# WinnerBy/PreGANPlus

Hardware: AMD Instinct MI355X
Metric: host-windows/sec (detect+diagnose+generate) (higher is better)
Workload: dtype fp32; 1 GPU; C2: PreGAN+ batched inference, 50 hosts x W=3 x 3 resources, 65536 windows per GPU, fp32; windows_per_gpu=65536, parallelism=dp1 (independent windows)

## Files before the change

### preganplus_amd/csrc/pgp_capi.hip

```cpp
#include <hip/hip_runtime.h>

#include <string>

#include "../../include/preganplus.h"
#include "pgp_device.hpp"
#include "pgp_pack.hpp"
#include "pgp_repack.hpp"
#include "pgp_train.hpp"
#include "pgp_tune.hpp"
#include "pgp_tunef.hpp"
#include "pgp_tunedp.hpp"

#include <vector>

using namespace pgp;

struct pgp_model {
  int H = 0, K = 0;
  bool fpe = false;
  bool loaded = false;
  float* d_frags = nullptr;
  float* d_decb = nullptr;
  float* d_encb = nullptr;
  bool enc_split = true;
  bool dec_split = true;
  float* d_ganb = nullptr;
  bool gan_split = true;
  float* d_tab = nullptr;
  float* d_gtab = nullptr;
  float* d_gat = nullptr;
  double* d_pscr = nullptr;
  int cap = 0;
  float* d_agg = nullptr;
  float* d_lat = nullptr;
  float* d_emb = nullptr;
};

namespace {
thread_local std::string g_err;
int fail(int code, const std::string& msg) {
  g_err = msg;
  return code;
}
#define HIPCHK(x)                                                                                  \
  do {                                                                                             \
    hipError_t e_ = (x);                                                                           \
    if (e_ != hipSuccess) return fail(PGP_ERR_HIP, std::string(#x) + ": " + hipGetErrorString(e_)); \
// ... 147 lines not shown
  if (batch < 0) return fail(PGP_ERR_ARG, "negative batch");
  if (stage < -1 || stage > 3) return fail(PGP_ERR_ARG, "bad stage");
  if (batch == 0) return PGP_OK;
  const bool all = stage == -1;
  if (((all || stage == 0) && !windows) ||
      ((all || stage == 2) && (!logits || !protos || !cls || !any_anom)) ||
      ((all || stage == 3) && (!sched || !probs || !keep_orig || !final_target || !gen_target)))
    return fail(PGP_ERR_ARG, "NULL input/output pointer");
  if (batch > m->cap) {
    const int rc = reserve(m, batch);
    if (rc) return rc;
  }
  FwdArgs a{};
  a.B = batch;
  a.H = m->H;
  a.K = m->K;
  a.windows = windows;
  a.sched = sched;
  a.agg = m->d_agg;
  a.lat = m->d_lat;
  a.emb = m->d_emb;
  a.frags = m->d_frags;
  a.decb = m->dec_split ? m->d_decb : nullptr;
  a.encb = m->enc_split ? m->d_encb : nullptr;
  a.ganb = m->gan_split ? m->d_ganb : nullptr;
  a.tab = m->d_tab;
  a.gtab = m->d_gtab;
  a.gat = m->d_gat;
  a.logits = logits;
  a.protos = protos;
  a.cls = cls;
  a.any_anom = any_anom;
  a.probs = probs;
  a.keep = keep_orig;
  a.final_t = final_target;
  a.gen_t = gen_target;
  a.latent = latent;
  hipStream_t st = reinterpret_cast<hipStream_t>(stream);
  if (all || stage == 0) HIPCHK(launch_gat(a, st));
  if (all || stage == 1) HIPCHK(launch_encoder(a, st));
  if (all || stage == 2) HIPCHK(launch_decoder(a, st));
  if (all || stage == 3) HIPCHK(launch_gan(a, st));
  return PGP_OK;
}

int pgp_forward(pgp_model* m, int batch, const float* windows, const float* sched, float* logits, float* protos,
                int* cls, int* any_anom, float* probs, int* keep_orig, int* final_target, int* gen_target,
                float* latent, void* stream) {
  return pgp_forward_stage(m, -1, batch, windows, sched, logits, protos, cls, any_anom, probs, keep_orig,
                           final_target, gen_target, latent, stream);
}

int pgp_forward_fpe_stage(pgp_model* m, int stage, int batch, const float* windows, const float* h0,
                          const float* sched, float* scores, float* protos, int* cls, int* any_anom, float* probs,
                          int* keep_orig, int* final_target, int* gen_target, void* stream) {
  if (!m) return fail(PGP_ERR_ARG, "NULL model");
  if (!m->loaded) return fail(PGP_ERR_STATE, "weights not loaded");
  if (!m->fpe) return fail(PGP_ERR_STATE, "not an FPE model: use pgp_forward");
  if (batch < 0) return fail(PGP_ERR_ARG, "negative batch");
  if (stage < -1 || stage > 1) return fail(PGP_ERR_ARG, "bad stage");
  if (batch == 0) return PGP_OK;
  const bool all = stage == -1;
  if (((all || stage == 0) && (!windows || !h0 || !scores || !protos || !cls || !any_anom)) ||
// ... 48 lines not shown
  HIPCHK(launch_decide(batch, n_hosts, keep_orig, final_target, cur_host, moves, hosts_from,
                       reinterpret_cast<hipStream_t>(stream)));
  return PGP_OK;
}

int pgp_embedding(int n_hosts, int batch, const float* logits, const float* protos, float* emb, void* stream) {
  if (n_hosts < 1 || batch < 0) return fail(PGP_ERR_ARG, "bad embedding arguments");
  if (batch == 0) return PGP_OK;
  if (!logits || !protos || !emb) return fail(PGP_ERR_ARG, "NULL input/output pointer");
  HIPCHK(launch_embed((long)batch * n_hosts, logits, protos, emb, reinterpret_cast<hipStream_t>(stream)));
  return PGP_OK;
}

int pgp_decoder_split(pgp_model* m, int on) {
  if (!m) return fail(PGP_ERR_ARG, "NULL model");
  if (m->fpe || decoder_split_floats(m->H) == 0)
    return on ? fail(PGP_ERR_UNSUPPORTED, "split-bf16 decoder not compiled for this model / host count") : PGP_OK;
  m->dec_split = on != 0;
  return PGP_OK;
}

int pgp_encoder_split(pgp_model* m, int on) {
  if (!m) return fail(PGP_ERR_ARG, "NULL model");
  if (m->fpe || encoder_split_floats(m->H) == 0)
    return on ? fail(PGP_ERR_UNSUPPORTED, "split-bf16 encoder not compiled for this model / host count") : PGP_OK;
  m->enc_split = on != 0;
  return PGP_OK;
}

int pgp_gan_split(pgp_model* m, int on) {
  if (!m) return fail(PGP_ERR_ARG, "NULL model");
  if (gan_split_floats(m->H) == 0)
    return on ? fail(PGP_ERR_UNSUPPORTED, "split-bf16 GAN kernel not compiled for this host count") : PGP_OK;
  m->gan_split = on != 0;
  return PGP_OK;
}

int pgp_schedule_onehot(int n_hosts, int batch, const unsigned char* idx, float* sched, void* stream) {
  if (n_hosts < 1 || n_hosts > 255 || batch < 0) return fail(PGP_ERR_ARG, "bad schedule_onehot arguments");
  if (batch == 0) return PGP_OK;
  if (!idx || !sched) return fail(PGP_ERR_ARG, "NULL input/output pointer");
  HIPCHK(launch_onehot(n_hosts, (long)batch * n_hosts, idx, sched, reinterpret_cast<hipStream_t>(stream)));
  return PGP_OK;
}

namespace {
bool master_offsets(int H, long* tr, long* gen, long* disc, long* all) {
  switch (H) {
#define CASE(h)                     \
// ... 415 lines not shown
```

### preganplus_amd/csrc/pgp_device.hpp

```cpp
#pragma once
#include <hip/hip_runtime.h>

#include <atomic>
#include <string>

#include "pgp_layout.hpp"

namespace pgp {

typedef float f32x4 __attribute__((ext_vector_type(4)));
typedef float f32x2 __attribute__((ext_vector_type(2)));

constexpr int kMaxProtos = 64;

inline int device_cus() {
  static std::atomic<int> cached[64];
  int dev = 0;
  if (hipGetDevice(&dev) != hipSuccess || dev < 0 || dev >= 64) return 256;
  int n = cached[dev].load(std::memory_order_relaxed);
  if (n == 0) {
    if (hipDeviceGetAttribute(&n, hipDeviceAttributeMultiprocessorCount, dev) != hipSuccess || n <= 0) n = 256;
    cached[dev].store(n, std::memory_order_relaxed);
  }
  return n;
// ... 29 lines not shown
  const float* windows;
  const float* h0;
  const float* tab;
  float* scores;
  float* protos;
  int* cls;
  int* any_anom;
  float* emb;
};
hipError_t launch_fpe(int H, const FpeArgs& a, hipStream_t st);
int fpe_param_count(int H);
hipError_t launch_fpe_step(int n_hosts, const float* win, const float* h0, const int* y, const int* cls,
                           const float* P, float* G, int K, double* state, double update_min, double decay,
                           double* loss, hipStream_t st);
hipError_t launch_fpe_forward_many(int n_hosts, int n, const float* wins, const float* h0s, const float* P,
                                   double* probs, double* protos, hipStream_t st);

hipError_t launch_decide(int B, int C, const int* keep, const int* target, const int* cur, int* moves,
                         int* hosts_from, hipStream_t st);
hipError_t launch_embed(long n, const float* logits, const float* protos, float* emb, hipStream_t st);
hipError_t launch_onehot(int H, long rows, const unsigned char* idx, float* sched, hipStream_t st);

hipError_t launch_gat(const FwdArgs& a, hipStream_t st);
hipError_t launch_encoder(const FwdArgs& a, hipStream_t st);
hipError_t launch_decoder(const FwdArgs& a, hipStream_t st);
long decoder_split_floats(int H);
hipError_t launch_decoder_split(int H, const float* frags, float* decb, hipStream_t st);
long encoder_split_floats(int H);
hipError_t launch_encoder_split(int H, const float* frags, float* encb, hipStream_t st);
hipError_t launch_gan(const FwdArgs& a, hipStream_t st);
long gan_split_floats(int H);
hipError_t launch_gan_split_derive(int H, const float* frags, float* planes, hipStream_t st);
hipError_t launch_gan_split(const FwdArgs& a, hipStream_t st);

struct AdamArgs;
struct AdamFuse;
long gan_workspace_floats(int H, int B);
int gan_plan_slices(int H, int B);
hipError_t launch_adamw(const AdamArgs& a, hipStream_t st);
bool gan1_supported(int H);
hipError_t launch_gan1_forward(int H, const float* emb, const float* sched, const float* Pg, const float* Pd,
                               float* row, float* ns, float* probs, hipStream_t st);
hipError_t launch_gan1_step(int H, const float* target, float* Pg, float* Pd, float* Gg, float* Gd, float* row,
                            const AdamArgs& ad, const AdamArgs& ag, float* probs_gen, float* probs_after,
                            hipStream_t st);

hipError_t launch_gan_fwd(int H, int B, const float* emb, const float* sched, const float* Pg, const float* Pd,
// ... 135 lines not shown
```

### preganplus_amd/csrc/pgp_encoder.hip

```cpp
#include "pgp_device.hpp"

namespace pgp {
namespace {

constexpr int kEncWaves = 4;
constexpr int kEnc16Waves = 4, kEnc16EU = 2;
template <int H>
constexpr bool tail_res() { return Geo<H>::TAIL; }
constexpr int kEncTailWaves = 8;
template <int H>
constexpr int enc_waves() { return H <= 16 ? kEnc16Waves : tail_res<H>() ? kEncTailWaves : kEncWaves; }
template <int H>
constexpr int NW_STAGE() { return enc_waves<H>(); }

#ifndef PGP_ENC_PIPE
#define PGP_ENC_PIPE 1
#endif
constexpr bool kEncPipe = PGP_ENC_PIPE != 0;
#ifndef PGP_ENC_PIPE_F32
#define PGP_ENC_PIPE_F32 0
#endif
constexpr bool kEncPipeF32 = PGP_ENC_PIPE_F32 != 0;

template <int H>
struct EncS {
  using G = Geo<H>;
  static constexpr int NBD = cdiv(G::KQ_D, 2);
  static constexpr int NBF = G::KQ_F / 2;
  static constexpr int F1S = G::MT_F * NBD * 3;
  static constexpr int F2S = G::MT_X * NBF * 3;
  static constexpr int FFN = F1S + F2S;
  static constexpr int L0F = 0;
  static constexpr int L1A = FFN;
  static constexpr int L1F = L1A + G::P_F1;
  static constexpr int GROUPS = L1F + FFN;
  static constexpr int STREAM = GROUPS * G::FQ;
  static constexpr long SIZE = STREAM;
};

template <int H, bool SPLIT = false>
struct EncLds {
  static constexpr bool TRES = tail_res<H>();
  static constexpr int RES0 = TRES ? Geo<H>::st_begin(Geo<H>::NST - 1) : 0;
  static constexpr int STREAM = SPLIT ? EncS<H>::STREAM : (kLayers * Geo<H>::LAYER_G - RES0) * Geo<H>::FQ;
  static constexpr bool RESIDENT = TRES || STREAM * 4 <= 32 * 1024;
// ... 112 lines not shown
        a = ld4(A + (m * KQ + q4) * 256 + lane * 4);
      }
      f32x4 rw[NR];
      if (m == 0) {
#pragma unroll
        for (int n = 0; n < NR; ++n) rw[n] = ld4(RW + ((n * KQ + q4) * 4 + g) * 4);
      }
#pragma unroll
      for (int e = 0; e < 4; ++e)
        if (4 * q4 + e < KS) {
#pragma unroll
          for (int w = 0; w < 3; ++w) {
            acc[m][w] = mfma(a[e], Bx[q4][w][e], acc[m][w]);
            if (m == 0) {
#pragma unroll
              for (int n = 0; n < NR; ++n) racc[n][w] = fmaf(rw[n][e], Bx[q4][w][e], racc[n][w]);
            }
          }
        }
    }
  prio_valu();
}

template <int NR>
PGP_DEV void rows_finish(float (&r)[NR][3]) {
  float* f = &r[0][0];
#pragma unroll
  for (int i = 0; i + 1 < 3 * NR; i += 2) xsum2(f[i], f[i + 1]);
  if constexpr ((3 * NR) % 2) f[3 * NR - 1] = xsum(f[3 * NR - 1], true);
}

template <int NR>
PGP_DEV float rows_pick(const float (&r)[NR][3], int w) {
  float v[NR];
#pragma unroll
  for (int n = 0; n < NR; ++n) v[n] = r[n][w];
  return xsum_rows<NR>(v);
}

template <int NR>
PGP_DEV void zero_rows(float (&r)[NR][3]) {
#pragma unroll
  for (int n = 0; n < NR; ++n)
#pragma unroll
    for (int w = 0; w < 3; ++w) r[n][w] = 0.f;
}
// ... 135 lines not shown
PGP_DEV void qkv_fold(f32x4 (&acc)[NM][3], int T0, int n, const float* tab, const float (&ba)[3], int lane, int g) {
  using G = Geo<H>;
#pragma unroll
  for (int m = 0; m < NM; ++m)
    if (m < n) {
      const float a = tab[G::T_F0 + (T0 + m) * 64 + lane];
#pragma unroll
      for (int w = 0; w < 3; ++w)
        acc[m][w] = mfma(a, ba[w], ld4(tab + G::T_F0B + (w * 3 * G::NQT + T0 + m) * 16 + 4 * g));
    }
}
template <int H>
PGP_DEV float row_fold_part(int m, int n, int w, const float* tab, const float (&ba)[3], int g) {
  using G = Geo<H>;
  const float t = tab[G::T_F0R + (m * G::SR + n) * 4 + g];
  return (g < 3 ? t : 0.f) * ba[w];
}
template <int H>
PGP_DEV float row_fold_bias(int m, int n, int w, const float* tab) {
  using G = Geo<H>;
  return tab[G::T_F0RB + w * 3 * G::SR + m * G::SR + n];
}

template <int H, bool F0, bool SPLIT>
PGP_DEV void encoder_layer_tail(f32x4 (&X)[Geo<H>::MT_D][3], Ring<H, SPLIT>& ring, const float* TL, int lane,
                                const float* tab, const float (&ba)[3], const float (&xv)[3][3]) {
  using G = Geo<H>;
  constexpr int TQ = G::TQ, SR = G::SR, HF = G::HF;
  const int g = lane >> 4;
  constexpr bool BIL = F0;
  f32x4 QK[BIL ? 1 : 2 * TQ][3];
  float qr[SR][3], kr[SR][3];
  if constexpr (BIL) {
  } else {
#pragma unroll
    for (int m = 0; m < 2 * TQ; ++m) {
      const f32x4 bias = ld4(TL + G::TL_QKV + m * 16 + 4 * g);
#pragma unroll
      for (int w = 0; w < 3; ++w) QK[m][w] = bias;
    }
    float qkr[2 * SR][3];
    zero_rows(qkr);
    gemm3_rows<2 * TQ, G::KQ_D, G::KS_D, G::MT_D, 2 * TQ, 2 * SR>(QK, ring.cur, X, lane, qkr, TL + G::TL_RQ, g);
    rows_finish(qkr);
#pragma unroll
    for (int n = 0; n < SR; ++n)
#pragma unroll
      for (int w = 0; w < 3; ++w) {
        qr[n][w] = qkr[n][w] + TL[G::TL_RQB + n];
        kr[n][w] = qkr[SR + n][w] + TL[G::TL_RQB + SR + n];
      }
  }
  ring.advance();
  float P0[3][3], P1[3][3];
  if constexpr (BIL) {
#pragma unroll
    for (int hh = 0; hh < 2; ++hh) {
      const float* SB = tab + G::T_F0S + hh * 36;
      float tk[3][3], vk[3][3];
#pragma unroll
      for (int w2 = 0; w2 < 3; ++w2) {
#pragma unroll
        for (int f = 0; f < 3; ++f)
          tk[w2][f] = fmaf(SB[3 * f + 2], xv[w2][2], fmaf(SB[3 * f + 1], xv[w2][1], fmaf(SB[3 * f], xv[w2][0], SB[9 + 3 * f + w2])));
#pragma unroll
        for (int w = 0; w < 3; ++w)
// ... 79 lines not shown
      for (int k = 0; k < 4; ++k)
#pragma unroll
        for (int mt = 0; mt < G::MT_X; ++mt)
          acc[mt][w] = mfma(tab[G::T_F0O + (k * G::MT_X + mt) * 64 + lane], bops[k], acc[mt][w]);
      float ro[G::XR];
#pragma unroll
      for (int n = 0; n < G::XR; ++n) {
        const float* rw = tab + G::T_F0OR + n * 16;
        ro[n] = g < 3 ? rw[g] * y0 + rw[4 + g] * p0 + rw[8 + g] * y1 + rw[12 + g] * p1 : 0.f;
      }
      acc[G::MT_X][w][0] += xsum_rows<G::XR>(ro);
    }
    layer_norm_tiles<H, false>(acc, X, TL + G::TL_LN1G, TL + G::TL_LN1B, g);
  } else {
  f32x4 V[TQ][3];
  float vr[SR][3];
#pragma unroll
  for (int t = 0; t < TQ; ++t) {
    const f32x4 bias = ld4(TL + G::TL_QKV + (2 * TQ + t) * 16 + 4 * g);
#pragma unroll
    for (int w = 0; w < 3; ++w) V[t][w] = bias;
  }
  zero_rows(vr);
  gemm3_rows<TQ, G::KQ_D, G::KS_D, G::MT_D, TQ, SR>(V, ring.cur, X, lane, vr, TL + G::TL_RQ + 2 * SR * G::KQ_D * 16,
                                                         g);
  float vd[3];
  {
    const float vb = TL[G::TL_RQB + 2 * SR + g];
#pragma unroll
    for (int w = 0; w < 3; ++w) vd[w] = rows_pick<SR>(vr, w) + (g < SR ? vb : 0.f);
  }
  f32x4 O[TQ + 1][3];
#pragma unroll
  for (int w = 0; w < 3; ++w) {
#pragma unroll
    for (int t = 0; t < 2 * HF; ++t) {
      const float(&Pw)[3][3] = t < HF ? P0 : P1;
      O[t][w] = Pw[w][0] * V[t][0] + Pw[w][1] * V[t][1] + Pw[w][2] * V[t][2];
    }
#pragma unroll
    for (int r = 0; r < 4; ++r) {
      const bool h0 = 4 * r + g < G::HT;
      const float c0 = h0 ? P0[w][0] : P1[w][0], c1 = h0 ? P0[w][1] : P1[w][1], c2 = h0 ? P0[w][2] : P1[w][2];
      O[2 * HF][w][r] = c0 * V[2 * HF][0][r] + c1 * V[2 * HF][1][r] + c2 * V[2 * HF][2][r];
    }
    const float o3 = P1[w][0] * vd[0] + P1[w][1] * vd[1] + P1[w][2] * vd[2];
    O[TQ][w] = f32x4{o3, 0.f, 0.f, 0.f};
  }
  {
    float ro[G::XR][3];
    zero_rows(ro);
    gemm3_rows<G::MT_X, G::KQ_OT, G::KS_OT, TQ + 1, G::MT_D, G::XR>(acc, ring.cur + G::G_V * G::FQ, O, lane, ro,
                                                                   TL + G::TL_RO, g);
#pragma unroll
    for (int w = 0; w < 3; ++w) acc[G::MT_X][w][0] += rows_pick<G::XR>(ro, w);
  }
  layer_norm_tiles<H, false>(acc, X, TL + G::TL_LN1G, TL + G::TL_LN1B, g);
  }
  ring.advance();
#pragma unroll
  for (int mt = 0; mt < G::MT_D; ++mt) {
    const f32x4 b2 = ld4(TL + G::TL_B2 + 16 * mt + 4 * g), g1 = ld4(TL + G::TL_LN1G + 16 * mt + 4 * g);
#pragma unroll
    for (int w = 0; w < 3; ++w) acc[mt][w] = X[mt][w] * g1 + b2;
  }
  if constexpr (SPLIT) {
    using S = EncS<H>;
    static_assert(S::NBF * 2 == G::MT_F, "hidden pairs");
    const float* A1 = ring.cur;
    const float* A2 = ring.cur + S::F1S * G::FQ;
#pragma unroll
    for (int w = 0; w < 3; ++w) {
      f32x4 F[G::MT_F];
#pragma unroll
      for (int c = 0; c < G::MT_F; ++c) F[c] = ld4(TL + G::TL_B1 + 16 * c + 4 * g);
      if constexpr (kEncPipe) {
// ... 197 lines not shown
  }
  gemm3<G::MT_F, G::KQ_D, G::KS_D, G::MT_D>(F1, ring.cur + G::G_O * G::FQ, X, lane);
#pragma unroll
  for (int mt = 0; mt < G::MT_F; ++mt)
#pragma unroll
    for (int w = 0; w < 3; ++w)
#pragma unroll
      for (int r = 0; r < 4; ++r) F1[mt][w][r] = relu_enc<H>(F1[mt][w][r]);
  ring.advance();
#pragma unroll
  for (int mt = 0; mt < G::MT_D; ++mt) {
    const f32x4 b2 = ld4(TL + G::TL_B2 + 16 * mt + 4 * g), g1 = ld4(TL + G::TL_LN1G + 16 * mt + 4 * g);
#pragma unroll
    for (int w = 0; w < 3; ++w) acc[mt][w] = X[mt][w] * g1 + b2;
  }
  gemm3<G::MT_D, G::KQ_F, 16, G::MT_F>(acc, ring.cur, F1, lane);
  ring.advance();
  layer_norm_tiles<H, false>(acc, X, TL + G::TL_LN2G, TL + G::TL_LN2B, g);
}

template <int H, bool SPLIT>
__global__ __launch_bounds__(enc_waves<H>() * 64, H <= 16 ? kEnc16EU : tail_res<H>() ? 1 : 2) void encoder_kernel(
    FwdArgs a) {
  using G = Geo<H>;
  using L = EncLds<H, SPLIT>;
  __shared__ __attribute__((aligned(16))) float smem[L::TOTAL];
  __shared__ float xstage[L::UNITS ? NW_STAGE<H>() * 144 : 1];
  float* tab = smem + (L::RESIDENT ? L::STREAM : 2 * L::SLOT);
  const int tsz = G::t_size(a.K);
  for (int i = threadIdx.x; i < tsz; i += blockDim.x) tab[i] = a.tab[i];

  const int lane = threadIdx.x & 63, g = lane >> 4, j = lane & 15;
  const int wv = __builtin_amdgcn_readfirstlane(threadIdx.x >> 6);
  constexpr int NW = enc_waves<H>();
  const long nblk = (a.B + 15) / 16;

  Ring<H, SPLIT> ring{smem, smem + L::SLOT, a.frags + G::OFF_ENC, 0, H * kLayers * G::NST, wv, lane};
  if constexpr (SPLIT) {
    dma_groups(a.encb, smem, EncS<H>::GROUPS, wv, NW, lane);
    ring.nxt = smem;
    ring.next = 1;
    __syncthreads();
  } else if constexpr (L::RESIDENT) {
    dma_groups(a.frags + G::OFF_ENC + (long)L::RES0 * G::FQ, smem, kLayers * G::LAYER_G - L::RES0, wv, NW, lane);
    ring.nxt = smem;
    ring.next = 1;
    __syncthreads();
  } else {
    ring.nxt = smem;
    ring.issue();
    ring.nxt = smem + L::SLOT;
    ring.next = 1;
    __syncthreads();
    ring.issue();
  }

  auto unit = [&](long blk, int h, bool active, const float* pre) {
    const float* agg = a.agg + (active ? blk : 0) * H * 3 * 48;
    float* lat = a.lat + (active ? blk : 0) * G::LAT_BLK;
    float ba[3];
    float xv[3][3];
    if constexpr (L::UNITS) {
#pragma unroll
      for (int w = 0; w < 3; ++w) {
#pragma unroll
        for (int f = 0; f < 3; ++f) xv[w][f] = G::TAIL ? pre[w * 48 + 16 * f + j] : 0.f;
        const float v = pre[w * 48 + (lane < 48 ? lane : 47)];
        ba[w] = g < 3 ? v : 0.f;
      }
    } else {
#pragma unroll
      for (int w = 0; w < 3; ++w) ba[w] = (active && g < 3) ? agg[(h * 3 + w) * 48 + lane] : 0.f;
#pragma unroll
      for (int w = 0; w < 3; ++w)
#pragma unroll
        for (int f = 0; f < 3; ++f)
          xv[w][f] = (G::TAIL && active) ? agg[(h * 3 + w) * 48 + 16 * f + j] : 0.f;
    }
    f32x4 X[G::MT_D][3];
#pragma unroll
    for (int mt = 0; mt < G::MT_D; ++mt) {
      const float aw = tab[G::T_TEW + mt * 64 + lane];
#pragma unroll
      for (int w = 0; w < 3; ++w) X[mt][w] = mfma(aw, ba[w], ld4(tab + G::T_TE + w * G::DP + 16 * mt + 4 * g));
    }
    static_assert(kLayers == 2, "layer 0 (folded q/k/v) + layer 1");
    if constexpr (G::TAIL) {
      encoder_layer_tail<H, true, SPLIT>(X, ring, tab + G::T_L0, lane, tab, ba, xv);
      encoder_layer_tail<H, false, SPLIT>(X, ring, tab + G::T_L0 + G::TL_SIZE, lane, tab, ba, xv);
    } else if constexpr (!SPLIT) {
      encoder_layer<H, true>(X, ring, tab + G::T_L0, lane, tab, ba);
      encoder_layer<H, false>(X, ring, tab + G::T_L0 + G::TL_SIZE, lane, tab, ba);
    }

    if (active) {
#pragma unroll
      for (int w = 0; w < 3; ++w) {
        float* lc = lat + (long)((h * 3 + w) * G::KS_D) * 64;
#pragma unroll
        for (int q = 0; q < G::LAT_FG; ++q) *reinterpret_cast<f32x4*>(lc + q * 256 + lane * 4) = X[q][w];
        if constexpr (G::KS_D % 4 != 0) {
#pragma unroll
          for (int r = 0; r < G::KS_D % 4; ++r) lc[G::LAT_FG * 256 + r * 64 + lane] = X[G::LAT_FG][w][r];
        }
      }
      if (a.latent != nullptr) {
        const long b = blk * 16 + j;
        if (b < a.B) {
#pragma unroll
          for (int w = 0; w < 3; ++w)
#pragma unroll
            for (int mt = 0; mt < G::MT_D; ++mt)
#pragma unroll
              for (int r = 0; r < 4; ++r) {
                const int c = 16 * mt + 4 * r + g;
                const float* TL1 = tab + G::T_L0 + G::TL_SIZE;
                if (c < H)
                  a.latent[b * G::LAT + (long)h * 3 * H + w * H + c] =
                      X[mt][w][r] * TL1[G::TL_LN2G + 16 * mt + 4 * g + r] + TL1[G::TL_LN2B + 16 * mt + 4 * g + r];
              }
        }
      }
    }
  };
  if constexpr (L::UNITS) {
    const long U = nblk * H, NWT = (long)gridDim.x * NW, gw = (long)blockIdx.x * NW + wv;
    const long u1 = (gw + 1) * U / NWT;
    float* slot = xstage + wv * 144;
    const long u0 = gw * U / NWT;
    float pf[3];
    auto load_x = [&](long u) {
#pragma unroll
      for (int k = 0; k < 3; ++k) pf[k] = a.agg[u * 144 + (64 * k + lane < 144 ? 64 * k + lane : 143)];
    };
    auto stage_x = [&]() {
#pragma unroll
      for (int k = 0; k < 3; ++k)
        if (64 * k + lane < 144) slot[64 * k + lane] = pf[k];
    };
    if (u0 < u1) {
      load_x(u0);
      stage_x();
    }
#pragma unroll 1
    for (long u = u0; u < u1; ++u) {
      load_x(u + 1 < u1 ? u + 1 : u);
      const long blk = u / H;
      unit(blk, (int)(u - blk * H), true, slot);
      stage_x();
    }
  } else {
    const long blk = (long)blockIdx.x * NW + wv;
    const bool active = blk < nblk;
#pragma unroll 1
    for (int h = 0; h < H; ++h) unit(blk, h, active, nullptr);
  }
}

template <int H, bool SPLIT>
hipError_t launch_form(const FwdArgs& a, hipStream_t st) {
  const long nblk = (a.B + 15) / 16;
  constexpr int NW = enc_waves<H>();
  long grid = (nblk + NW - 1) / NW;
  static std::atomic<int> fits{-1};
  if (fits.load(std::memory_order_relaxed) < 0) {
    hipFuncAttributes fa{};
    const bool ok = hipFuncGetAttributes(&fa, reinterpret_cast<const void*>(encoder_kernel<H, SPLIT>)) == hipSuccess &&
                    fa.maxThreadsPerBlock >= NW * 64;
    fits.store(ok ? 1 : 0, std::memory_order_relaxed);
  }
  if (!fits.load(std::memory_order_relaxed)) return hipErrorLaunchOutOfResources;
  if constexpr (EncLds<H>::UNITS) {
    static std::atomic<int> occ_cache{0};
    int occ = occ_cache.load(std::memory_order_relaxed);
    if (occ <= 0) {
      if (hipOccupancyMaxActiveBlocksPerMultiprocessor(&occ, encoder_kernel<H, SPLIT>, NW * 64, 0) != hipSuccess ||
          occ <= 0)
        occ = 1;
      occ_cache.store(occ, std::memory_order_relaxed);
    }
    grid = std::min<long>((long)device_cus() * occ, (nblk * H + NW - 1) / NW);
  }
  encoder_kernel<H, SPLIT><<<(int)grid, NW * 64, 0, st>>>(a);
  return hipGetLastError();
}

template <int H>
hipError_t launch(const FwdArgs& a, hipStream_t st) {
  if constexpr (enc_split<H>())
    if (a.encb != nullptr) return launch_form<H, true>(a, st);
  return launch_form<H, false>(a, st);
}

template <int H>
hipError_t launch_split(const float* frags, float* encb, hipStream_t st) {
  if constexpr (enc_split<H>()) {
    using G = Geo<H>;
    constexpr long n = 2L * (G::MT_F * EncS<H>::NBD + G::MT_X * EncS<H>::NBF) + G::P_F1;
    enc_split_kernel<H><<<(int)((n + 3) / 4), 256, 0, st>>>(frags + G::OFF_ENC, encb);
    return hipGetLastError();
  }
  return hipErrorInvalidValue;
}

}

hipError_t launch_encoder(const FwdArgs& a, hipStream_t st) {
  switch (a.H) {
#define CASE(h) \
  case h:       \
    return launch<h>(a, st);
    PGP_FOR_EACH_H(CASE)
#undef CASE
  }
  return hipErrorInvalidValue;
}

long encoder_split_floats(int H) {
  switch (H) {
#define CASE(h) \
  case h:       \
    return enc_split<h>() ? EncS<h>::SIZE : 0;
    PGP_FOR_EACH_H(CASE)
#undef CASE
  }
  return 0;
}

hipError_t launch_encoder_split(int H, const float* frags, float* encb, hipStream_t st) {
  switch (H) {
#define CASE(h) \
  case h:       \
    return launch_split<h>(frags, encb, st);
    PGP_FOR_EACH_H(CASE)
// ... 7 lines not shown
```

### preganplus_amd/model.py

```python
from __future__ import annotations

import ctypes

import numpy as np
import torch

from . import _native
from . import weights as W


class DecisionModel:
    def __init__(self, n_hosts: int, weights: dict, device: str | torch.device = "cuda"):
        self.H = int(n_hosts)
        self.K = int(np.asarray(weights["prototypes"]).shape[0])
        self.device = torch.device(device)
        if self.device.type == "cuda" and self.device.index is None:
            self.device = torch.device("cuda", torch.cuda.current_device())
        if self.device.type != "cuda":
            raise ValueError("DecisionModel runs on the GPU only (no CPU fallback)")
        L = _native.lib()
        if self.H not in _native.supported_hosts():
            raise ValueError(f"H={self.H} not compiled in; supported {_native.supported_hosts()}")
        self._L = L
        h = ctypes.c_void_p()
# ... 21 lines not shown
                                                pr.ctypes.data_as(ctypes.POINTER(ctypes.c_double))),
                      "pgp_load_weights_master")
        self.prototypes = pr.copy()

    def repack_master(self, P: torch.Tensor, protos_dev: torch.Tensor, prototypes_host=None, stream=None,
                      sections: int = 3):
        if protos_dev.dtype != torch.float64 or protos_dev.numel() != 2 * self.K or not protos_dev.is_contiguous():
            raise ValueError(f"protos_dev must be contiguous float64 [{self.K},2] on the device")
        L = self._L
        L.pgp_repack_master_sections.argtypes = [ctypes.c_void_p] * 3 + [ctypes.c_int, ctypes.c_void_p]
        st = stream if stream is not None else torch.cuda.current_stream(self.device)
        _native.check(L.pgp_repack_master_sections(self._h, ctypes.c_void_p(P.data_ptr()),
                                                   ctypes.c_void_p(protos_dev.data_ptr()), int(sections),
                                                   ctypes.c_void_p(st.cuda_stream)), "pgp_repack_master_sections")
        if prototypes_host is not None:
            self.prototypes = np.array(prototypes_host, dtype=np.float64)

    def reserve(self, max_batch: int):
        _native.check(self._L.pgp_reserve(self._h, int(max_batch)), "pgp_reserve")

    def gan_split(self, on: bool):
        _native.check(self._L.pgp_gan_split(self._h, int(bool(on))), "pgp_gan_split")

    def encoder_split(self, on: bool):
        _native.check(self._L.pgp_encoder_split(self._h, int(bool(on))), "pgp_encoder_split")

    def decoder_split(self, on: bool):
        _native.check(self._L.pgp_decoder_split(self._h, int(bool(on))), "pgp_decoder_split")

    def alloc_outputs(self, B: int, latent: bool = False, packed: bool = False):
        dev, H = self.device, self.H
        f32, i32 = torch.float32, torch.int32
        spec = [("logits", f32, (B, H, 2)), ("protos", f32, (B, H, 2)), ("cls", i32, (B, H)), ("any", i32, (B,)),
                ("probs", f32, (B, 2)), ("keep", i32, (B,)), ("final_target", i32, (B, H)),
                ("gen_target", i32, (B, H))]
        if packed:
            n = sum(int(np.prod(s)) for _, _, s in spec)
            buf = torch.zeros(n, dtype=i32, device=dev)
            out, o = {}, 0
            for name, dt, shp in spec:
                k = int(np.prod(shp))
                out[name] = buf[o:o + k].view(dt).view(shp)
                o += k
            out["_buf"] = buf
            out["_hbuf"] = torch.zeros(n, dtype=i32).pin_memory()
        else:
            out = {name: torch.empty(shp, dtype=dt, device=dev) for name, dt, shp in spec}
        out["latent"] = torch.empty((B, 3 * H * H), dtype=f32, device=dev) if latent else None
# ... 157 lines not shown
```

### preganplus_amd/roofline.py

```python
from __future__ import annotations

PEAK_FP32_TFLOPS = 157.3
PEAK_HBM_GBS = 8000.0
PEAK_BF16_TFLOPS = 2500.0

W = 3
FF = 64
GAN_HIDDEN = 64


def macs_per_window(H: int) -> dict:
    d = H
    tokens = W * H
    hd = d // 2
    gat = tokens * 3 * d + 2 * tokens * d + W * H * H * d
    te = tokens * d * d
    per_token_layer = 3 * d * d + d * d + 2 * (W * hd) * 2 + 2 * FF * d
    layers = 2 * tokens * per_token_layer
    dec = (W * H * d) * (4 * H)
    gan = GAN_HIDDEN * (2 * H + H * H) + (H * H) * GAN_HIDDEN + GAN_HIDDEN * 2 * H * H + 2 * GAN_HIDDEN
    return dict(gat=gat, time_encoder=te, encoder_layers=layers, decoders=dec, gan=gan)


def flops_per_window(H: int) -> dict:
# ... 5 lines not shown


def encdec_flops_per_window(H: int) -> int:
    f = flops_per_window(H)
    return f["time_encoder"] + f["encoder_layers"] + f["decoders"]


def encoder_flops_per_window(H: int) -> int:
    f = flops_per_window(H)
    return f["time_encoder"] + f["encoder_layers"]


ENC_MFMA_PER_HOST = {16: 264, 50: 1116}


def encoder_executed_flops_per_window(H: int):
    n = ENC_MFMA_PER_HOST.get(H)
    return None if n is None else n * 2048 * H / 16


ENC_SPLIT_MFMA_PER_HOST = {50: (516, 504)}


def encoder_split(H: int) -> bool:
    return H in ENC_SPLIT_MFMA_PER_HOST


def encoder_split_executed_flops_per_window(H: int):
    f32, bf = ENC_SPLIT_MFMA_PER_HOST[H]
    return f32 * 2048 * H / 16, bf * 16 * 16 * 32 * 2 * H / 16


TUNE_MFMA_PER_UNIT = {
    16: {"tf_fwd_kernel": 156, "tf_bwd_ffn_kernel": 288, "tf_bwd_att_kernel": 96},
    50: {"tf_fwd_kernel": 840, "tf_bwd_ffn_kernel": 384, "tf_bwd_att_kernel": 1200},
}
TUNE_BF16_PER_UNIT = {
    16: {"tf_fwd_kernel": 0, "tf_bwd_ffn_kernel": 0, "tf_bwd_att_kernel": 0},
    50: {"tf_fwd_kernel": 288, "tf_bwd_ffn_kernel": 576, "tf_bwd_att_kernel": 144},
}
TUNE_FUSED_LAUNCHES = ("fwd layer 0", "fwd layer 1", "ffn bwd layer 1", "att bwd layer 1", "ffn bwd layer 0",
                       "att bwd layer 0")


def tf_grid(units: int, waves: int, cus: int, reserve: int = 0) -> int:
    r = max(0, min(reserve, cus // 2))
    gmax = max(1, min(cus - r, (units + waves - 1) // waves))
    m = (units + waves * gmax - 1) // (waves * gmax)
    return max(1, (units + waves * m - 1) // (waves * m))


def tune_fused_grids(H: int, B: int, B_fwd: int | None, cus: int, reserve: int = 0):
# ... 108 lines not shown
```

Measured before the change: 654.1 million host-windows/s.

## Add split-bf16 attention GEMM encoder form with pipelined A-fragment loads

Adds a new encoder kernel variant (form 1, now the default) for layer 1 of the tail encoder. Its V and output-projection GEMMs run as split-bf16 MFMA (bf16x6 emulation of fp32) instead of fp32 MFMA, and it prefetches the next A fragments ahead of each MFMA. The kernel body moves into a shared include so both variants compile from one source, and the new kernel uses launch bounds of one block per EU. This trades fp32 MFMA throughput for more bf16 MFMAs plus split overhead and register pressure, and it risks lower occupancy.

Measured after the change: 662.7 million host-windows/s (median of 6 runs). No clear change (+1.3%).

```diff
diff --git a/preganplus_amd/csrc/pgp_capi.hip b/preganplus_amd/csrc/pgp_capi.hip
--- a/preganplus_amd/csrc/pgp_capi.hip
+++ b/preganplus_amd/csrc/pgp_capi.hip
@@ -22,7 +22,7 @@
   float* d_frags = nullptr;
   float* d_decb = nullptr;
   float* d_encb = nullptr;
-  bool enc_split = true;
+  int enc_split = 1;
   bool dec_split = true;
   float* d_ganb = nullptr;
   bool gan_split = true;
@@ -216,7 +216,7 @@
   a.emb = m->d_emb;
   a.frags = m->d_frags;
   a.decb = m->dec_split ? m->d_decb : nullptr;
-  a.encb = m->enc_split ? m->d_encb : nullptr;
+  a.encb = m->enc_split != 0 ? m->d_encb : nullptr;
   a.ganb = m->gan_split ? m->d_ganb : nullptr;
   a.tab = m->d_tab;
   a.gtab = m->d_gtab;
@@ -232,7 +232,7 @@
   a.latent = latent;
   hipStream_t st = reinterpret_cast<hipStream_t>(stream);
   if (all || stage == 0) HIPCHK(launch_gat(a, st));
-  if (all || stage == 1) HIPCHK(launch_encoder(a, st));
+  if (all || stage == 1) HIPCHK(launch_encoder(a, st, m->enc_split));
   if (all || stage == 2) HIPCHK(launch_decoder(a, st));
   if (all || stage == 3) HIPCHK(launch_gan(a, st));
   return PGP_OK;
@@ -327,9 +327,10 @@
 
 int pgp_encoder_split(pgp_model* m, int on) {
   if (!m) return fail(PGP_ERR_ARG, "NULL model");
+  if (on < 0 || on > 2) return fail(PGP_ERR_ARG, "encoder form must be 0, 1 or 2");
   if (m->fpe || encoder_split_floats(m->H) == 0)
     return on ? fail(PGP_ERR_UNSUPPORTED, "split-bf16 encoder not compiled for this model / host count") : PGP_OK;
-  m->enc_split = on != 0;
+  m->enc_split = on;
   return PGP_OK;
 }
 
diff --git a/preganplus_amd/csrc/pgp_device.hpp b/preganplus_amd/csrc/pgp_device.hpp
--- a/preganplus_amd/csrc/pgp_device.hpp
+++ b/preganplus_amd/csrc/pgp_device.hpp
@@ -75,7 +75,7 @@
 hipError_t launch_onehot(int H, long rows, const unsigned char* idx, float* sched, hipStream_t st);
 
 hipError_t launch_gat(const FwdArgs& a, hipStream_t st);
-hipError_t launch_encoder(const FwdArgs& a, hipStream_t st);
+hipError_t launch_encoder(const FwdArgs& a, hipStream_t st, int form);
 hipError_t launch_decoder(const FwdArgs& a, hipStream_t st);
 long decoder_split_floats(int H);
 hipError_t launch_decoder_split(int H, const float* frags, float* decb, hipStream_t st);
diff --git a/preganplus_amd/csrc/pgp_encoder.hip b/preganplus_amd/csrc/pgp_encoder.hip
--- a/preganplus_amd/csrc/pgp_encoder.hip
+++ b/preganplus_amd/csrc/pgp_encoder.hip
@@ -21,6 +21,22 @@
 #define PGP_ENC_PIPE_F32 0
 #endif
 constexpr bool kEncPipeF32 = PGP_ENC_PIPE_F32 != 0;
+#ifndef PGP_ENC_ATT_QK
+#define PGP_ENC_ATT_QK 0
+#endif
+#ifndef PGP_ENC_ATT_V
+#define PGP_ENC_ATT_V 1
+#endif
+#ifndef PGP_ENC_ATT_O
+#define PGP_ENC_ATT_O 1
+#endif
+#ifndef PGP_ENC_ATT_PIPE
+#define PGP_ENC_ATT_PIPE 1
+#endif
+constexpr bool kEncAttPipe = PGP_ENC_ATT_PIPE != 0;
+
+constexpr int kAttQK = 1, kAttV = 2, kAttO = 4;
+constexpr int kEncAtt = (PGP_ENC_ATT_QK ? kAttQK : 0) | (PGP_ENC_ATT_V ? kAttV : 0) | (PGP_ENC_ATT_O ? kAttO : 0);
 
 template <int H>
 struct EncS {
@@ -179,6 +195,75 @@
   prio_valu();
 }
 
+template <int NM, int KS, int NB, int NMA, int NR, bool PIPE = true>
+PGP_DEV void gemm3_rows_split(f32x4 (&acc)[NMA][3], const float* A, const f32x4 (&Bx)[NB][3], int lane,
+                              float (&racc)[NR][3], const float* RW, int g) {
+  constexpr int KQ = 4, NBLK = KQ / 2, QN = NBLK * NM;
+  static_assert(NM <= NMA && NB == KQ && KS <= 4 * KQ, "accumulator tiles, two 32-k blocks");
+  prio_mfma();
+  f32x4 an0, an1;
+  if constexpr (PIPE) {
+    an0 = ld4(A + lane * 4);
+    an1 = ld4(A + 256 + lane * 4);
+  }
+#pragma unroll
+  for (int b = 0; b < NBLK; ++b) {
+    u32x4 xb[3][3];
+#pragma unroll
+    for (int w = 0; w < 3; ++w) {
+      float v[8];
+      pair_tiles<NB>(Bx, b, w, v);
+      split8(v, xb[w]);
+    }
+#pragma unroll
+    for (int m = 0; m < NM; ++m) {
+      f32x4 a0, a1;
+      if constexpr (PIPE) {
+        a0 = an0;
+        a1 = an1;
+        const int q = b * NM + m + 1;
+        if (q < QN) {
+          an0 = ld4(A + ((q % NM) * KQ + 2 * (q / NM)) * 256 + lane * 4);
+          an1 = ld4(A + ((q % NM) * KQ + 2 * (q / NM) + 1) * 256 + lane * 4);
+        }
+        __builtin_amdgcn_sched_barrier(0);
+      } else {
+        a0 = ld4(A + (m * KQ + 2 * b) * 256 + lane * 4);
+        a1 = ld4(A + (m * KQ + 2 * b + 1) * 256 + lane * 4);
+      }
+      u32x4 wp[3];
+      {
+        float v[8];
+#pragma unroll
+        for (int e = 0; e < 4; ++e) {
+          v[e] = a0[e];
+          v[4 + e] = a1[e];
+        }
+        split8(v, wp);
+      }
+      if (m == 0) {
+#pragma unroll
+        for (int q4 = 2 * b; q4 < 2 * b + 2; ++q4) {
+          f32x4 rw[NR];
+#pragma unroll
+          for (int n = 0; n < NR; ++n) rw[n] = ld4(RW + ((n * KQ + q4) * 4 + g) * 4);
+#pragma unroll
+          for (int e = 0; e < 4; ++e)
+            if (4 * q4 + e < KS) {
+#pragma unroll
+              for (int w = 0; w < 3; ++w)
+#pragma unroll
+                for (int n = 0; n < NR; ++n) racc[n][w] = fmaf(rw[n][e], Bx[q4][w][e], racc[n][w]);
+            }
+        }
+      }
+#pragma unroll
+      for (int w = 0; w < 3; ++w) acc[m][w] = mfma_bf6(wp, xb[w], acc[m][w]);
+    }
+  }
+  prio_valu();
+}
+
 template <int NR>
 PGP_DEV void rows_finish(float (&r)[NR][3]) {
   float* f = &r[0][0];
@@ -360,12 +445,13 @@
   return tab[G::T_F0RB + w * 3 * G::SR + m * G::SR + n];
 }
 
-template <int H, bool F0, bool SPLIT>
+template <int H, bool F0, bool SPLIT, int ATT = 0>
 PGP_DEV void encoder_layer_tail(f32x4 (&X)[Geo<H>::MT_D][3], Ring<H, SPLIT>& ring, const float* TL, int lane,
                                 const float* tab, const float (&ba)[3], const float (&xv)[3][3]) {
   using G = Geo<H>;
   constexpr int TQ = G::TQ, SR = G::SR, HF = G::HF;
   const int g = lane >> 4;
+  static_assert(ATT == 0 || (SPLIT && !F0 && G::KQ_D == 4 && G::KQ_OT == 4), "split attention GEMMs: layer 1, two 32-k blocks");
   constexpr bool BIL = F0;
   f32x4 QK[BIL ? 1 : 2 * TQ][3];
   float qr[SR][3], kr[SR][3];
@@ -379,7 +465,10 @@
     }
     float qkr[2 * SR][3];
     zero_rows(qkr);
-    gemm3_rows<2 * TQ, G::KQ_D, G::KS_D, G::MT_D, 2 * TQ, 2 * SR>(QK, ring.cur, X, lane, qkr, TL + G::TL_RQ, g);
+    if constexpr ((ATT & kAttQK) != 0)
+      gemm3_rows_split<2 * TQ, G::KS_D, G::MT_D, 2 * TQ, 2 * SR, kEncAttPipe>(QK, ring.cur, X, lane, qkr, TL + G::TL_RQ, g);
+    else
+      gemm3_rows<2 * TQ, G::KQ_D, G::KS_D, G::MT_D, 2 * TQ, 2 * SR>(QK, ring.cur, X, lane, qkr, TL + G::TL_RQ, g);
     rows_finish(qkr);
 #pragma unroll
     for (int n = 0; n < SR; ++n)
@@ -505,8 +594,11 @@
     for (int w = 0; w < 3; ++w) V[t][w] = bias;
   }
   zero_rows(vr);
-  gemm3_rows<TQ, G::KQ_D, G::KS_D, G::MT_D, TQ, SR>(V, ring.cur, X, lane, vr, TL + G::TL_RQ + 2 * SR * G::KQ_D * 16,
-                                                         g);
+  if constexpr ((ATT & kAttV) != 0)
+    gemm3_rows_split<TQ, G::KS_D, G::MT_D, TQ, SR, kEncAttPipe>(V, ring.cur, X, lane, vr, TL + G::TL_RQ + 2 * SR * G::KQ_D * 16, g);
+  else
+    gemm3_rows<TQ, G::KQ_D, G::KS_D, G::MT_D, TQ, SR>(V, ring.cur, X, lane, vr, TL + G::TL_RQ + 2 * SR * G::KQ_D * 16,
+                                                           g);
   float vd[3];
   {
     const float vb = TL[G::TL_RQB + 2 * SR + g];
@@ -533,8 +625,12 @@
   {
     float ro[G::XR][3];
     zero_rows(ro);
-    gemm3_rows<G::MT_X, G::KQ_OT, G::KS_OT, TQ + 1, G::MT_D, G::XR>(acc, ring.cur + G::G_V * G::FQ, O, lane, ro,
-                                                                   TL + G::TL_RO, g);
+    if constexpr ((ATT & kAttO) != 0)
+      gemm3_rows_split<G::MT_X, G::KS_OT, TQ + 1, G::MT_D, G::XR, kEncAttPipe>(acc, ring.cur + G::G_V * G::FQ, O, lane, ro,
+                                                                 TL + G::TL_RO, g);
+    else
+      gemm3_rows<G::MT_X, G::KQ_OT, G::KS_OT, TQ + 1, G::MT_D, G::XR>(acc, ring.cur + G::G_V * G::FQ, O, lane, ro,
+                                                                     TL + G::TL_RO, g);
 #pragma unroll
     for (int w = 0; w < 3; ++w) acc[G::MT_X][w][0] += rows_pick<G::XR>(ro, w);
   }
@@ -778,150 +874,33 @@
 template <int H, bool SPLIT>
 __global__ __launch_bounds__(enc_waves<H>() * 64, H <= 16 ? kEnc16EU : tail_res<H>() ? 1 : 2) void encoder_kernel(
     FwdArgs a) {
-  using G = Geo<H>;
-  using L = EncLds<H, SPLIT>;
-  __shared__ __attribute__((aligned(16))) float smem[L::TOTAL];
-  __shared__ float xstage[L::UNITS ? NW_STAGE<H>() * 144 : 1];
-  float* tab = smem + (L::RESIDENT ? L::STREAM : 2 * L::SLOT);
-  const int tsz = G::t_size(a.K);
-  for (int i = threadIdx.x; i < tsz; i += blockDim.x) tab[i] = a.tab[i];
-
-  const int lane = threadIdx.x & 63, g = lane >> 4, j = lane & 15;
-  const int wv = __builtin_amdgcn_readfirstlane(threadIdx.x >> 6);
-  constexpr int NW = enc_waves<H>();
-  const long nblk = (a.B + 15) / 16;
-
-  Ring<H, SPLIT> ring{smem, smem + L::SLOT, a.frags + G::OFF_ENC, 0, H * kLayers * G::NST, wv, lane};
-  if constexpr (SPLIT) {
-    dma_groups(a.encb, smem, EncS<H>::GROUPS, wv, NW, lane);
-    ring.nxt = smem;
-    ring.next = 1;
-    __syncthreads();
-  } else if constexpr (L::RESIDENT) {
-    dma_groups(a.frags + G::OFF_ENC + (long)L::RES0 * G::FQ, smem, kLayers * G::LAYER_G - L::RES0, wv, NW, lane);
-    ring.nxt = smem;
-    ring.next = 1;
-    __syncthreads();
-  } else {
-    ring.nxt = smem;
-    ring.issue();
-    ring.nxt = smem + L::SLOT;
-    ring.next = 1;
-    __syncthreads();
-    ring.issue();
-  }
-
-  auto unit = [&](long blk, int h, bool active, const float* pre) {
-    const float* agg = a.agg + (active ? blk : 0) * H * 3 * 48;
-    float* lat = a.lat + (active ? blk : 0) * G::LAT_BLK;
-    float ba[3];
-    float xv[3][3];
-    if constexpr (L::UNITS) {
-#pragma unroll
-      for (int w = 0; w < 3; ++w) {
-#pragma unroll
-        for (int f = 0; f < 3; ++f) xv[w][f] = G::TAIL ? pre[w * 48 + 16 * f + j] : 0.f;
-        const float v = pre[w * 48 + (lane < 48 ? lane : 47)];
-        ba[w] = g < 3 ? v : 0.f;
-      }
-    } else {
-#pragma unroll
-      for (int w = 0; w < 3; ++w) ba[w] = (active && g < 3) ? agg[(h * 3 + w) * 48 + lane] : 0.f;
-#pragma unroll
-      for (int w = 0; w < 3; ++w)
-#pragma unroll
-        for (int f = 0; f < 3; ++f)
-          xv[w][f] = (G::TAIL && active) ? agg[(h * 3 + w) * 48 + 16 * f + j] : 0.f;
-    }
-    f32x4 X[G::MT_D][3];
-#pragma unroll
-    for (int mt = 0; mt < G::MT_D; ++mt) {
-      const float aw = tab[G::T_TEW + mt * 64 + lane];
-#pragma unroll
-      for (int w = 0; w < 3; ++w) X[mt][w] = mfma(aw, ba[w], ld4(tab + G::T_TE + w * G::DP + 16 * mt + 4 * g));
-    }
-    static_assert(kLayers == 2, "layer 0 (folded q/k/v) + layer 1");
-    if constexpr (G::TAIL) {
-      encoder_layer_tail<H, true, SPLIT>(X, ring, tab + G::T_L0, lane, tab, ba, xv);
-      encoder_layer_tail<H, false, SPLIT>(X, ring, tab + G::T_L0 + G::TL_SIZE, lane, tab, ba, xv);
-    } else if constexpr (!SPLIT) {
-      encoder_layer<H, true>(X, ring, tab + G::T_L0, lane, tab, ba);
-      encoder_layer<H, false>(X, ring, tab + G::T_L0 + G::TL_SIZE, lane, tab, ba);
-    }
-
-    if (active) {
-#pragma unroll
-      for (int w = 0; w < 3; ++w) {
-        float* lc = lat + (long)((h * 3 + w) * G::KS_D) * 64;
-#pragma unroll
-        for (int q = 0; q < G::LAT_FG; ++q) *reinterpret_cast<f32x4*>(lc + q * 256 + lane * 4) = X[q][w];
-        if constexpr (G::KS_D % 4 != 0) {
-#pragma unroll
-          for (int r = 0; r < G::KS_D % 4; ++r) lc[G::LAT_FG * 256 + r * 64 + lane] = X[G::LAT_FG][w][r];
-        }
-      }
-      if (a.latent != nullptr) {
-        const long b = blk * 16 + j;
-        if (b < a.B) {
-#pragma unroll
-          for (int w = 0; w < 3; ++w)
-#pragma unroll
-            for (int mt = 0; mt < G::MT_D; ++mt)
-#pragma unroll
-              for (int r = 0; r < 4; ++r) {
-                const int c = 16 * mt + 4 * r + g;
-                const float* TL1 = tab + G::T_L0 + G::TL_SIZE;
-                if (c < H)
-                  a.latent[b * G::LAT + (long)h * 3 * H + w * H + c] =
-                      X[mt][w][r] * TL1[G::TL_LN2G + 16 * mt + 4 * g + r] + TL1[G::TL_LN2B + 16 * mt + 4 * g + r];
-              }
-        }
-      }
-    }
-  };
-  if constexpr (L::UNITS) {
-    const long U = nblk * H, NWT = (long)gridDim.x * NW, gw = (long)blockIdx.x * NW + wv;
-    const long u1 = (gw + 1) * U / NWT;
-    float* slot = xstage + wv * 144;
-    const long u0 = gw * U / NWT;
-    float pf[3];
-    auto load_x = [&](long u) {
-#pragma unroll
-      for (int k = 0; k < 3; ++k) pf[k] = a.agg[u * 144 + (64 * k + lane < 144 ? 64 * k + lane : 143)];
-    };
-    auto stage_x = [&]() {
-#pragma unroll
-      for (int k = 0; k < 3; ++k)
-        if (64 * k + lane < 144) slot[64 * k + lane] = pf[k];
-    };
-    if (u0 < u1) {
-      load_x(u0);
-      stage_x();
-    }
-#pragma unroll 1
-    for (long u = u0; u < u1; ++u) {
-      load_x(u + 1 < u1 ? u + 1 : u);
-      const long blk = u / H;
-      unit(blk, (int)(u - blk * H), true, slot);
-      stage_x();
-    }
-  } else {
-    const long blk = (long)blockIdx.x * NW + wv;
-    const bool active = blk < nblk;
-#pragma unroll 1
-    for (int h = 0; h < H; ++h) unit(blk, h, active, nullptr);
-  }
-}
-
-template <int H, bool SPLIT>
+  constexpr int ATT = 0;
+#include "pgp_encoder_body.inc"
+}
+
+template <int H>
+__global__ __launch_bounds__(enc_waves<H>() * 64, 1) void encoder_att_kernel(FwdArgs a) {
+  constexpr bool SPLIT = true;
+  constexpr int ATT = kEncAtt;
+#include "pgp_encoder_body.inc"
+}
+
+template <int H, int FORM>
 hipError_t launch_form(const FwdArgs& a, hipStream_t st) {
+  constexpr bool SPLIT = FORM != 0;
+  const auto kern = [] {
+    if constexpr (FORM == 1)
+      return encoder_att_kernel<H>;
+    else
+      return encoder_kernel<H, SPLIT>;
+  }();
   const long nblk = (a.B + 15) / 16;
   constexpr int NW = enc_waves<H>();
   long grid = (nblk + NW - 1) / NW;
   static std::atomic<int> fits{-1};
   if (fits.load(std::memory_order_relaxed) < 0) {
     hipFuncAttributes fa{};
-    const bool ok = hipFuncGetAttributes(&fa, reinterpret_cast<const void*>(encoder_kernel<H, SPLIT>)) == hipSuccess &&
+    const bool ok = hipFuncGetAttributes(&fa, reinterpret_cast<const void*>(kern)) == hipSuccess &&
                     fa.maxThreadsPerBlock >= NW * 64;
     fits.store(ok ? 1 : 0, std::memory_order_relaxed);
   }
@@ -930,22 +909,22 @@
     static std::atomic<int> occ_cache{0};
     int occ = occ_cache.load(std::memory_order_relaxed);
     if (occ <= 0) {
-      if (hipOccupancyMaxActiveBlocksPerMultiprocessor(&occ, encoder_kernel<H, SPLIT>, NW * 64, 0) != hipSuccess ||
+      if (hipOccupancyMaxActiveBlocksPerMultiprocessor(&occ, kern, NW * 64, 0) != hipSuccess ||
           occ <= 0)
         occ = 1;
       occ_cache.store(occ, std::memory_order_relaxed);
     }
     grid = std::min<long>((long)device_cus() * occ, (nblk * H + NW - 1) / NW);
   }
-  encoder_kernel<H, SPLIT><<<(int)grid, NW * 64, 0, st>>>(a);
+  kern<<<(int)grid, NW * 64, 0, st>>>(a);
   return hipGetLastError();
 }
 
 template <int H>
-hipError_t launch(const FwdArgs& a, hipStream_t st) {
+hipError_t launch(const FwdArgs& a, hipStream_t st, int form) {
   if constexpr (enc_split<H>())
-    if (a.encb != nullptr) return launch_form<H, true>(a, st);
-  return launch_form<H, false>(a, st);
+    if (a.encb != nullptr && form != 0) return form == 2 ? launch_form<H, 2>(a, st) : launch_form<H, 1>(a, st);
+  return launch_form<H, 0>(a, st);
 }
 
 template <int H>
@@ -961,11 +940,11 @@
 
 }
 
-hipError_t launch_encoder(const FwdArgs& a, hipStream_t st) {
+hipError_t launch_encoder(const FwdArgs& a, hipStream_t st, int form) {
   switch (a.H) {
 #define CASE(h) \
   case h:       \
-    return launch<h>(a, st);
+    return launch<h>(a, st, form);
     PGP_FOR_EACH_H(CASE)
 #undef CASE
   }
diff --git a/preganplus_amd/csrc/pgp_encoder_body.inc b/preganplus_amd/csrc/pgp_encoder_body.inc
--- /dev/null
+++ b/preganplus_amd/csrc/pgp_encoder_body.inc
@@ -0,0 +1,133 @@
+  using G = Geo<H>;
+  using L = EncLds<H, SPLIT>;
+  __shared__ __attribute__((aligned(16))) float smem[L::TOTAL];
+  __shared__ float xstage[L::UNITS ? NW_STAGE<H>() * 144 : 1];
+  float* tab = smem + (L::RESIDENT ? L::STREAM : 2 * L::SLOT);
+  const int tsz = G::t_size(a.K);
+  for (int i = threadIdx.x; i < tsz; i += blockDim.x) tab[i] = a.tab[i];
+
+  const int lane = threadIdx.x & 63, g = lane >> 4, j = lane & 15;
+  const int wv = __builtin_amdgcn_readfirstlane(threadIdx.x >> 6);
+  constexpr int NW = enc_waves<H>();
+  const long nblk = (a.B + 15) / 16;
+
+  Ring<H, SPLIT> ring{smem, smem + L::SLOT, a.frags + G::OFF_ENC, 0, H * kLayers * G::NST, wv, lane};
+  if constexpr (SPLIT) {
+    dma_groups(a.encb, smem, EncS<H>::GROUPS, wv, NW, lane);
+    ring.nxt = smem;
+    ring.next = 1;
+    __syncthreads();
+  } else if constexpr (L::RESIDENT) {
+    dma_groups(a.frags + G::OFF_ENC + (long)L::RES0 * G::FQ, smem, kLayers * G::LAYER_G - L::RES0, wv, NW, lane);
+    ring.nxt = smem;
+    ring.next = 1;
+    __syncthreads();
+  } else {
+    ring.nxt = smem;
+    ring.issue();
+    ring.nxt = smem + L::SLOT;
+    ring.next = 1;
+    __syncthreads();
+    ring.issue();
+  }
+
+  auto unit = [&](long blk, int h, bool active, const float* pre) {
+    const float* agg = a.agg + (active ? blk : 0) * H * 3 * 48;
+    float* lat = a.lat + (active ? blk : 0) * G::LAT_BLK;
+    float ba[3];
+    float xv[3][3];
+    if constexpr (L::UNITS) {
+#pragma unroll
+      for (int w = 0; w < 3; ++w) {
+#pragma unroll
+        for (int f = 0; f < 3; ++f) xv[w][f] = G::TAIL ? pre[w * 48 + 16 * f + j] : 0.f;
+        const float v = pre[w * 48 + (lane < 48 ? lane : 47)];
+        ba[w] = g < 3 ? v : 0.f;
+      }
+    } else {
+#pragma unroll
+      for (int w = 0; w < 3; ++w) ba[w] = (active && g < 3) ? agg[(h * 3 + w) * 48 + lane] : 0.f;
+#pragma unroll
+      for (int w = 0; w < 3; ++w)
+#pragma unroll
+        for (int f = 0; f < 3; ++f)
+          xv[w][f] = (G::TAIL && active) ? agg[(h * 3 + w) * 48 + 16 * f + j] : 0.f;
+    }
+    f32x4 X[G::MT_D][3];
+#pragma unroll
+    for (int mt = 0; mt < G::MT_D; ++mt) {
+      const float aw = tab[G::T_TEW + mt * 64 + lane];
+#pragma unroll
+      for (int w = 0; w < 3; ++w) X[mt][w] = mfma(aw, ba[w], ld4(tab + G::T_TE + w * G::DP + 16 * mt + 4 * g));
+    }
+    static_assert(kLayers == 2, "layer 0 (folded q/k/v) + layer 1");
+    if constexpr (G::TAIL) {
+      encoder_layer_tail<H, true, SPLIT>(X, ring, tab + G::T_L0, lane, tab, ba, xv);
+      encoder_layer_tail<H, false, SPLIT, ATT>(X, ring, tab + G::T_L0 + G::TL_SIZE, lane, tab, ba, xv);
+    } else if constexpr (!SPLIT) {
+      encoder_layer<H, true>(X, ring, tab + G::T_L0, lane, tab, ba);
+      encoder_layer<H, false>(X, ring, tab + G::T_L0 + G::TL_SIZE, lane, tab, ba);
+    }
+
+    if (active) {
+#pragma unroll
+      for (int w = 0; w < 3; ++w) {
+        float* lc = lat + (long)((h * 3 + w) * G::KS_D) * 64;
+#pragma unroll
+        for (int q = 0; q < G::LAT_FG; ++q) *reinterpret_cast<f32x4*>(lc + q * 256 + lane * 4) = X[q][w];
+        if constexpr (G::KS_D % 4 != 0) {
+#pragma unroll
+          for (int r = 0; r < G::KS_D % 4; ++r) lc[G::LAT_FG * 256 + r * 64 + lane] = X[G::LAT_FG][w][r];
+        }
+      }
+      if (a.latent != nullptr) {
+        const long b = blk * 16 + j;
+        if (b < a.B) {
+#pragma unroll
+          for (int w = 0; w < 3; ++w)
+#pragma unroll
+            for (int mt = 0; mt < G::MT_D; ++mt)
+#pragma unroll
+              for (int r = 0; r < 4; ++r) {
+                const int c = 16 * mt + 4 * r + g;
+                const float* TL1 = tab + G::T_L0 + G::TL_SIZE;
+                if (c < H)
+                  a.latent[b * G::LAT + (long)h * 3 * H + w * H + c] =
+                      X[mt][w][r] * TL1[G::TL_LN2G + 16 * mt + 4 * g + r] + TL1[G::TL_LN2B + 16 * mt + 4 * g + r];
+              }
+        }
+      }
+    }
+  };
+  if constexpr (L::UNITS) {
+    const long U = nblk * H, NWT = (long)gridDim.x * NW, gw = (long)blockIdx.x * NW + wv;
+    const long u1 = (gw + 1) * U / NWT;
+    float* slot = xstage + wv * 144;
+    const long u0 = gw * U / NWT;
+    float pf[3];
+    auto load_x = [&](long u) {
+#pragma unroll
+      for (int k = 0; k < 3; ++k) pf[k] = a.agg[u * 144 + (64 * k + lane < 144 ? 64 * k + lane : 143)];
+    };
+    auto stage_x = [&]() {
+#pragma unroll
+      for (int k = 0; k < 3; ++k)
+        if (64 * k + lane < 144) slot[64 * k + lane] = pf[k];
+    };
+    if (u0 < u1) {
+      load_x(u0);
+      stage_x();
+    }
+#pragma unroll 1
+    for (long u = u0; u < u1; ++u) {
+      load_x(u + 1 < u1 ? u + 1 : u);
+      const long blk = u / H;
+      unit(blk, (int)(u - blk * H), true, slot);
+      stage_x();
+    }
+  } else {
+    const long blk = (long)blockIdx.x * NW + wv;
+    const bool active = blk < nblk;
+#pragma unroll 1
+    for (int h = 0; h < H; ++h) unit(blk, h, active, nullptr);
+  }
diff --git a/preganplus_amd/model.py b/preganplus_amd/model.py
--- a/preganplus_amd/model.py
+++ b/preganplus_amd/model.py
@@ -67,8 +67,9 @@
     def gan_split(self, on: bool):
         _native.check(self._L.pgp_gan_split(self._h, int(bool(on))), "pgp_gan_split")
 
-    def encoder_split(self, on: bool):
-        _native.check(self._L.pgp_encoder_split(self._h, int(bool(on))), "pgp_encoder_split")
+    def encoder_split(self, on: bool, form: int | None = None):
+        f = int(bool(on)) if form is None else int(form)
+        _native.check(self._L.pgp_encoder_split(self._h, f), "pgp_encoder_split")
 
     def decoder_split(self, on: bool):
         _native.check(self._L.pgp_decoder_split(self._h, int(bool(on))), "pgp_decoder_split")
diff --git a/preganplus_amd/roofline.py b/preganplus_amd/roofline.py
--- a/preganplus_amd/roofline.py
+++ b/preganplus_amd/roofline.py
@@ -51,12 +51,16 @@
 ENC_SPLIT_MFMA_PER_HOST = {50: (516, 504)}
 
 
+ENC_ATT_SPLIT_TILES = {50: 6}
+ENC_ATT_MFMA_PER_HOST = {50: (282, 720)}
+
+
 def encoder_split(H: int) -> bool:
     return H in ENC_SPLIT_MFMA_PER_HOST
 
 
 def encoder_split_executed_flops_per_window(H: int):
-    f32, bf = ENC_SPLIT_MFMA_PER_HOST[H]
+    f32, bf = ENC_ATT_MFMA_PER_HOST.get(H) or ENC_SPLIT_MFMA_PER_HOST[H]
     return f32 * 2048 * H / 16, bf * 16 * 16 * 32 * 2 * H / 16
 
 
```
